# alshai/pfbwt-f

Hardware: AMD Instinct MI355X
Metric: Gbases/s end-to-end BWT+SA build; bit-exact .bwt/.sa vs reference (higher is better)
Workload: dtype u8 text / u32 indices / u64 hash; 1 GPU; S-32G; L=32000000, H=1000, seed=1000, w=10, p=100, flags=-r, uint_t=64, n=32000010000, r=83625322, input=text resident in HBM, outputs (.bwt, .ssa, .esa) left in HBM, per_rank=single GPU

## Files before the change

### include/pfbwt_hip_dev.h

```cpp
#ifndef PFBWT_HIP_DEV_H
#define PFBWT_HIP_DEV_H
#include "pfbwt_hip.h"

#ifdef __cplusplus
extern "C" {
#endif

int pfp_profile_enable(pfp_ctx *ctx, int on);
int pfp_profile_select(pfp_ctx *ctx, const char *kernel_name);
int pfp_profile_reset(pfp_ctx *ctx);
int pfp_profile_get(pfp_ctx *ctx, int idx, const char **name, uint64_t *launches, double *ms, double *bytes);
int pfp_stage_ms(pfp_ctx *ctx, double out[3]);
int pfp_debug_set(pfp_ctx *ctx, const char *key, long long value);
int pfp_debug_sort(pfp_ctx *ctx, uint64_t n, int bits, int reps, double *ms_out, uint32_t *unsorted_pairs, uint32_t *wrong_values);

int pfp_debug_prims_geometry(uint32_t out[4]);
int pfp_debug_sort_pairs(pfp_ctx *ctx, const void *keys, int key_bytes, const uint32_t *vals, uint64_t n, const int *ranges, int nranges,
                         void *keys_out, uint32_t *vals_out, uint32_t *guards_changed);
int pfp_debug_scan(pfp_ctx *ctx, const void *in, int elem_bytes, int op, int mode, uint64_t n, void *out, void *total, uint32_t *guards_changed);
int pfp_debug_compact(pfp_ctx *ctx, const uint32_t *in, const uint32_t *flag, uint64_t n, uint32_t *out, uint32_t *count, uint32_t *guards_changed);
int pfp_debug_checksum(pfp_ctx *ctx, const void *d_buf, uint64_t bytes, uint64_t global_offset, uint64_t out[2]);

int pfp_debug_check_sample_order(pfp_ctx *ctx, uint64_t out[5]);
int pfp_debug_check_sa(pfp_ctx *ctx, uint64_t out[5]);
int pfp_debug_check_samples(pfp_ctx *ctx, uint64_t out[3]);
int pfp_debug_rows_windowed(pfp_ctx *ctx, uint64_t window_rows, void *host_sa, void *host_lcp);
int pfp_debug_wordsum(pfp_ctx *ctx, const void *d_buf, uint64_t bytes, uint64_t out[2]);

#ifdef __cplusplus
}
#endif
#endif
```

### pfbwt-f_amd/csrc/common.h

```cpp
#pragma once
#include <hip/hip_runtime.h>
#include <cstdint>
#include <cstdio>
#include <cstdlib>
#include <cstring>
#include <chrono>
#include <string>
#include <vector>
#include "../../include/pfbwt_hip.h"
#include "devmem.h"
#include "../../include/pfbwt_hip_dev.h"

namespace pfp {

typedef uint32_t idx_t;

constexpr int BLOCK = 256;
constexpr int WAVE = 64;

constexpr uint8_t Dollar = 2, EndOfWord = 1, EndOfDict = 0;

enum KernelId {
    K_TRIGGER_SCAN, K_PHRASE_ENDS, K_PHRASE_HASH, K_PHRASE_HASH_LONG, K_DEDUP_HEADS, K_DEDUP_LONG,
    K_DICT_BUILD, K_RADIX_HIST, K_RADIX_SCATTER, K_SCAN_REDUCE, K_SCAN_SPINE, K_SCAN_APPLY,
// ... 157 lines not shown
    pfp::ResultSlot ms; uint64_t ms_patterns = 0, ms_bases = 0;
    std::vector<uint64_t> ms_off;
    pfp::ResultSlot rii; pfp::RiIndex rix;
    pfp::ResultSlot ri; uint64_t ri_patterns = 0, ri_reported = 0; int ri_route = 0;
    std::vector<uint64_t> ri_off;
    pfp::ResultSlot mem; uint64_t mem_patterns = 0, mem_count = 0;
    pfp::ResultSlot meml; uint64_t mem_reported = 0;
    std::vector<uint64_t> mem_off, mem_poff;
    size_t lo_after_parse = 0, lo_after_pbwt = 0, emit_scratch_mark = 0;
    bool prof_on = false; uint64_t prof_mask = ~0ULL;
    pfp::ProfRec prof[pfp::K_COUNT_];
    struct PendingEv { hipEvent_t a, b; int id; double bytes; };
    std::vector<PendingEv> pending;
    std::vector<hipEvent_t> ev_pool;
    double stage_ms[3] = {0, 0, 0};
    int hip_err = 0;
    uint8_t *hstage[2] = {nullptr, nullptr}; hipEvent_t hstage_ev[2] = {nullptr, nullptr}; bool hstage_used[2] = {false, false};
    pfp::Tunables tun;
    struct FastaIngest {
        uint8_t *raw[2] = {nullptr, nullptr}; size_t rawcap = 0; bool used[2] = {false, false};
        hipStream_t copy = nullptr; bool copy_ready = false; hipEvent_t ev_copied[2] = {nullptr, nullptr}, ev_free[2] = {nullptr, nullptr};
        uint8_t *tiles = nullptr; size_t tiles_cap = 0;
        unsigned long long *d_tot = nullptr, *h_tot = nullptr;
        uint32_t state = 2; bool started = false; uint64_t records = 0;
        std::vector<uint64_t> rec_raw, rec_pos;
    } fa;
    uint8_t *h_bwt = nullptr; void *h_sa = nullptr;
    uint8_t *ing_buf[16] = {};
    uint64_t ing_next_off = 0;
    std::vector<std::string> doc_names; std::vector<uint64_t> doc_starts;
    uint64_t hash_seed = 0x9E3779B97F4A7C15ULL;
    int num_cus = 0;
    uint32_t *d_trigtab = nullptr;
};

namespace pfp {

inline hipEvent_t ev_get(pfp_ctx *c)
{
    if (!c->ev_pool.empty()) { hipEvent_t e = c->ev_pool.back(); c->ev_pool.pop_back(); return e; }
    hipEvent_t e; (void)hipEventCreate(&e); return e;
}
inline void prof_collect(pfp_ctx *c)
{
    if (c->pending.empty()) return;
    (void)hipStreamSynchronize(c->stream);
    for (auto &pe : c->pending) {
        float ms = 0; (void)hipEventElapsedTime(&ms, pe.a, pe.b);
        c->prof[pe.id].launches++; c->prof[pe.id].ms += ms; c->prof[pe.id].bytes += pe.bytes;
        c->ev_pool.push_back(pe.a); c->ev_pool.push_back(pe.b);
    }
    c->pending.clear();
}
struct ProfScope {
    pfp_ctx *c; int id; double bytes; hipEvent_t a = nullptr; bool on = false;
    ProfScope(pfp_ctx *c_, int id_, double bytes_) : c(c_), id(id_), bytes(bytes_)
    {
        on = c->prof_on && ((c->prof_mask >> id) & 1ULL);
        if (on) { a = ev_get(c); (void)hipEventRecord(a, c->stream); }
    }
    ~ProfScope()
    {
        if (on) {
            hipEvent_t b = ev_get(c); (void)hipEventRecord(b, c->stream);
            c->pending.push_back({a, b, id, bytes});
            if (c->pending.size() > 4096) prof_collect(c);
// ... 68 lines not shown
```

### pfbwt-f_amd/csrc/emit.h

```cpp
#pragma once
#include "prims.h"
#include "parse.h"

namespace pfp {

__global__ __launch_bounds__(BLOCK) void k_pbwt_pack(const uint32_t *P, const uint8_t *last, const tpos_t *sai, uint64_t m, uint4 *rec)
{
    const uint64_t j = (uint64_t)blockIdx.x * BLOCK + threadIdx.x;
    if (j >= m) return;
    const uint64_t v = sai ? (uint64_t)sai[j] : 0ULL;
    rec[j] = make_uint4((uint32_t)v, (uint32_t)(v >> 32), P[j], (uint32_t)last[j ? j - 1 : m - 1]);
}
constexpr int BWL_SHIFT = 29;
__device__ __forceinline__ uint32_t bwl_code(uint32_t c) { return c == 0 ? 0u : c == Dollar ? 1u : c == '-' ? 2u : c == 'A' ? 3u : c == 'C' ? 4u : c == 'G' ? 5u : c == 'N' ? 6u : c == 'T' ? 7u : 8u; }
__device__ __forceinline__ uint8_t bwl_byte(uint32_t code) { return code == 0 ? (uint8_t)0 : code == 1 ? Dollar : code == 2 ? (uint8_t)'-' : code == 3 ? (uint8_t)'A' : code == 4 ? (uint8_t)'C' : code == 5 ? (uint8_t)'G' : code == 6 ? (uint8_t)'N' : (uint8_t)'T'; }
__global__ __launch_bounds__(BLOCK) void k_pbwt_rows(const uint32_t *SAP, const uint4 *rec, uint64_t m, uint8_t *bwlast, tpos_t *bwsai, uint32_t *W, uint32_t *rowid, int pack, uint32_t *bad)
{
    const uint64_t i = (uint64_t)blockIdx.x * BLOCK + threadIdx.x;
    if (i > m) return;
    const uint32_t s = SAP[i];
    if (s == 0) { bwlast[i] = 0; if (bwsai) bwsai[i] = 0; W[i] = 0; rowid[i] = (uint32_t)i; return; }
    const uint4 R = rec[s - 1];
    bwlast[i] = (uint8_t)R.w;
    if (bwsai) bwsai[i] = (tpos_t)(((uint64_t)R.y << 32) | R.x);
// ... 103 lines not shown
    const uint32_t *srank = nullptr;
    const tpos_t *bwsai = nullptr;
    const uint2 *posinfo = nullptr;
    const uint4 *prec = nullptr;
    const uint32_t *wordid = nullptr;
    int use_prec = 0;
    int use_e0 = 0;
    const uint4 *winfo = nullptr;
    const uint8_t *bwlast = nullptr;
    const uint8_t *bwl_il = nullptr;
    const tpos_t *bwsai_il = nullptr;
    const void *EB = nullptr;
    const uint32_t *s_sl = nullptr;
    const uint32_t *s_fb = nullptr;
    const uint8_t *s_fl = nullptr;
    const uint8_t *s_pc = nullptr;
    const uint32_t *s_g0 = nullptr;
    const uint32_t *gk = nullptr;
    const void *cnt = nullptr;
    const uint4 *sinfo = nullptr;
    const uint32_t *tile_slot = nullptr;
    uint64_t *big_keys = nullptr; uint32_t *big_vals = nullptr; unsigned long long *big_count = nullptr;
    uint64_t big_cap = 0, big_total = 0;
    uint64_t nout = 0, n = 0;
    uint64_t e0 = 0, e1 = 0;
    uint64_t w0 = 0, w1 = 0;
    const void *ENB = nullptr; const uint32_t *etile_slot = nullptr, *elist = nullptr, *cpos = nullptr; uint32_t ecount = 0; int special = 0; uint64_t q0 = 0;
    const uint32_t *qspec = nullptr;
    const uint32_t *gqf = nullptr, *gql = nullptr;
    uint8_t *gleft = nullptr, *tile_left = nullptr; uint32_t group_rows_cap = 0; uint32_t rank_members_max = 0;
    const uint4 *cinfo = nullptr;
    const unsigned long long *cgb = nullptr;
    const uint32_t *town = nullptr;
    uint32_t *lglist = nullptr; unsigned long long *lgcount = nullptr; uint64_t lgcap = 0; int qpasses = 0 ;
    unsigned long long *gstat = nullptr;
};
constexpr uint8_t SF_MULTI = 1, SF_FULL = 2, SF_BIG = 4, SF_GFULL = 8, SF_NONUNI = 16, SF_E0 = 32;
__device__ __forceinline__ bool slot_is_special(uint32_t fl) { return (fl & (SF_FULL | SF_GFULL | SF_NONUNI)) != 0; }
constexpr int EG_SLOTS = 2 * BLOCK;
constexpr uint32_t BIG_GROUP_MEMBERS = 64;
constexpr uint32_t WID_MASK = 0x0FFFFFFFu;
__device__ __forceinline__ uint32_t dict_code4(uint32_t c) { return c <= 2 ? c : (c == '-') ? 3u : (c == 'A') ? 4u : (c == 'C') ? 5u : (c == 'G') ? 6u : (c == 'N') ? 7u : 8u; }
__device__ __forceinline__ uint8_t dict_byte4(uint32_t code) { return code <= 2 ? (uint8_t)code : code == 3 ? (uint8_t)'-' : code == 4 ? (uint8_t)'A' : code == 5 ? (uint8_t)'C' : code == 6 ? (uint8_t)'G' : code == 7 ? (uint8_t)'N' : (uint8_t)'T'; }
__global__ __launch_bounds__(BLOCK) void k_pack_winfo(const uint32_t *ws, const uint32_t *wrank , const uint32_t *occ, const uint32_t *F, uint64_t dwords, uint4 *winfo)
{
    const uint64_t id = (uint64_t)blockIdx.x * BLOCK + threadIdx.x;
    if (id >= dwords) return;
    const uint32_t rk = wrank ? wrank[id] : (uint32_t)id;
    winfo[id] = make_uint4(ws[id], ws[id + 1] - 1u, F[rk], occ[rk]);
}
__global__ __launch_bounds__(BLOCK) void k_pack_posinfo(const uint8_t *D, const uint32_t *wordid, uint64_t dsize, uint2 *posinfo)
{
    const uint64_t x = (uint64_t)blockIdx.x * BLOCK + threadIdx.x;
    if (x >= dsize) return;
    posinfo[x] = make_uint2(wordid[x] | (dict_code4(x ? D[x - 1] : 0u) << 28), 0u);
}

constexpr uint32_t PREC_SL_BITS = 26, PREC_FULL = 1u << 30, PREC_VALID = 1u << 31;
__global__ __launch_bounds__(BLOCK) void k_pack_prec(const uint8_t *D, const uint32_t *wordid, const uint4 *winfo, uint64_t dsize, uint32_t dwords, uint4 *prec, const tpos_t *bwsai_il )
{
    const uint64_t x = (uint64_t)blockIdx.x * BLOCK + threadIdx.x;
    if (x >= dsize) return;
    const uint32_t id = wordid[x];
    uint4 R = make_uint4(0u, 0u, 0u, 0u);
    if (id < dwords) {
        const uint4 W = winfo[id];
        uint32_t code = 0, full = 0;
// ... 619 lines not shown
            }
        }
#pragma unroll
        for (int it = 0; it < EG_PER_THREAD; ++it) {
            const uint32_t r = threadIdx.x + (uint32_t)it * BLOCK;
            if (r < nrows) { LQ[r] = qv[it]; const uint32_t fl = s_kf[sv[it]] >> 24; if (fl & SF_MULTI) cv[it] = s_pc[sv[it]]; else if (!a.bwl_il) cv[it] = a.bwlast[qv[it]]; }
        }
        __syncthreads();
#pragma unroll
        for (int it = 0; it < EG_PER_THREAD; ++it) {
            const uint32_t r = threadIdx.x + (uint32_t)it * BLOCK;
            if (r < nrows) {
                const uint32_t s = sv[it], kf = s_kf[s];
                uint32_t pos = r;
                if ((kf >> 24) & SF_MULTI) {
                    const uint32_t sh = s - s_dl[s], k = kf & 0xFFFFFFu, q = qv[it];
                    uint32_t before = 0;
                    for (uint32_t mm = 0; mm < k; ++mm) {
                        const uint32_t sm = sh + mm;
                        if (sm != s) before += lower_bound_u32(LQ + s_eb[sm], s_eb[sm + 1] - s_eb[sm], q);
                    }
                    pos = s_eb[sh] + before + (r - s_eb[s]);
                }
                if (qrow) qrow[B0 - a.q0 + pos] = qv[it];
                const uint64_t o = s_ob[s] + pos;
                if (o >= a.w0 && o < a.w1) bwt[o - a.w0] = cv[it];
            }
        }
        __syncthreads();
        j += cut;
    }
}

template <int ITEMS> __device__ __forceinline__ void lds_sort_pairs_u32(uint32_t *keys, uint16_t *vals, uint32_t n, int npass, uint32_t (*wh)[RS_RADIX], uint32_t *red)
{
    const int lane = threadIdx.x & 63, wave = threadIdx.x >> 6;
    const uint32_t nit = (n + BLOCK - 1) / BLOCK;
    for (uint32_t j = n + threadIdx.x; j < nit * BLOCK; j += BLOCK) { keys[j] = 0xFFFFFFFFu; vals[j] = 0; }
    const uint32_t base = (uint32_t)wave * (nit * WAVE) + lane;
    for (int p = 0; p < npass; ++p) {
        const int sh = 8 * p;
        uint32_t k[ITEMS], dg[ITEMS]; uint16_t v[ITEMS];
#pragma unroll
        for (int w = 0; w < BLOCK / WAVE; ++w) wh[w][threadIdx.x] = 0;
        __syncthreads();
#pragma unroll
        for (int it = 0; it < ITEMS; ++it) {
            if ((uint32_t)it < nit) {
                const uint32_t i = base + (uint32_t)it * WAVE;
                k[it] = keys[i]; v[it] = vals[i];
                const uint32_t d = (k[it] >> sh) & 255u;
                uint32_t plo = 0xFFFFFFFFu, phi = 0xFFFFFFFFu;
                same_digit_lanes(d, plo, phi);
                const int leader = plo ? __builtin_ctz(plo) : 32 + __builtin_ctz(phi);
                uint32_t old = 0;
                if (lane == leader) { old = wh[wave][d]; wh[wave][d] = old + (uint32_t)__builtin_popcount(plo) + (uint32_t)__builtin_popcount(phi); }
                old = __shfl(old, leader);
                dg[it] = d | ((old + __builtin_amdgcn_mbcnt_hi(phi, __builtin_amdgcn_mbcnt_lo(plo, 0u))) << 8);
            }
        }
        __syncthreads();
        {
            const unsigned d = threadIdx.x;
            uint32_t cw[BLOCK / WAVE]; uint32_t total = 0;
#pragma unroll
            for (int w = 0; w < BLOCK / WAVE; ++w) { cw[w] = wh[w][d]; total += cw[w]; }
            uint32_t tt;
            uint32_t run = block_excl_sum(total, red, &tt);
#pragma unroll
            for (int w = 0; w < BLOCK / WAVE; ++w) { wh[w][d] = run; run += cw[w]; }
        }
        __syncthreads();
#pragma unroll
        for (int it = 0; it < ITEMS; ++it) {
            if ((uint32_t)it < nit) { const uint32_t li = wh[wave][dg[it] & 255u] + (dg[it] >> 8); keys[li] = k[it]; vals[li] = v[it]; }
        }
        __syncthreads();
    }
}
template <typename EBT, int BUF> __global__ __launch_bounds__(BLOCK) void k_emit_groups_large(EmitArgs a, uint8_t *bwt, uint32_t *qrow)
{
    __shared__ uint32_t LQ[BUF];
    __shared__ uint16_t LS[BUF];
    __shared__ uint32_t wh[BLOCK / WAVE][RS_RADIX];
    __shared__ uint32_t s_eb[EG_SLOTS + 1], s_fb[EG_SLOTS];
    __shared__ uint8_t s_pc[EG_SLOTS];
    __shared__ uint32_t red[4];
    const EBT *ENB = reinterpret_cast<const EBT *>(a.ENB);
    constexpr int WHICH = BUF > EG1_BUF ? 1 : 0;
    const unsigned long long have = a.lgcount[WHICH];
    const uint64_t cnt = have < a.lgcap ? have : a.lgcap;
    for (uint64_t g = blockIdx.x; g < cnt; g += gridDim.x) {
        const uint64_t j = a.lglist[(uint64_t)WHICH * a.lgcap + g];
        const uint32_t k = a.cinfo[j].y;
        const uint64_t B0 = (uint64_t)ENB[j], outbase = (uint64_t)a.cgb[j];
        for (uint32_t s = threadIdx.x; s < k; s += BLOCK) {
            const uint4 ci = a.cinfo[j + s];
            s_eb[s] = (uint32_t)((uint64_t)ENB[j + s] - B0); s_fb[s] = ci.x; s_pc[s] = (uint8_t)ci.w;
            if (s + 1 == k) s_eb[k] = (uint32_t)((uint64_t)ENB[j + k] - B0);
        }
        __syncthreads();
        const uint32_t nrows = s_eb[k];
        for (uint32_t r = threadIdx.x; r < nrows; r += BLOCK) { const uint32_t s = upper_bound_t<uint32_t>(s_eb, k, r) - 1u; LQ[r] = a.ilist[s_fb[s] + (r - s_eb[s])]; LS[r] = (uint16_t)s; }
        __syncthreads();
        lds_sort_pairs_u32<BUF / BLOCK>(LQ, LS, nrows, a.qpasses, wh, red);
        for (uint32_t r = threadIdx.x; r < nrows; r += BLOCK) {
            if (qrow) qrow[B0 - a.q0 + r] = LQ[r];
            const uint64_t o = outbase + r;
            if (o >= a.w0 && o < a.w1) bwt[o - a.w0] = s_pc[LS[r]];
        }
        __syncthreads();
    }
}

template <typename EBT> __global__ __launch_bounds__(BLOCK) void k_slice_bounds(EmitArgs a, uint64_t lo, uint64_t hi, unsigned long long *out)
{
    if (blockIdx.x != 0 || threadIdx.x != 0) return;
    const EBT *EB = reinterpret_cast<const EBT *>(a.EB);
    const EBT *ENB = reinterpret_cast<const EBT *>(a.ENB);
    const uint32_t il = slot_of_row<EBT>(a, lo);
    const uint32_t gh = (a.s_fl[il] & SF_MULTI) ? a.s_g0[il] : il;
    out[0] = EB[gh];
    out[2] = a.special ? (unsigned long long)ENB[a.cpos[gh]] : 0ULL;
    out[4] = a.special ? (unsigned long long)a.cpos[gh] : 0ULL;
    if (hi >= a.nout) { out[1] = a.nout; out[3] = a.special ? (unsigned long long)ENB[a.ecount] : 0ULL; out[5] = a.special ? (unsigned long long)a.ecount : 0ULL; return; }
    uint32_t s = slot_of_row<EBT>(a, hi - 1);
    if (a.s_fl[s] & SF_MULTI) { const uint32_t g = a.s_g0[s]; while (s < a.dsize && (a.s_fl[s] & SF_MULTI) && a.s_g0[s] == g) ++s; }
    else ++s;
    {
        uint64_t lo_ = s, hi_ = a.dsize;
        while (lo_ < hi_) { const uint64_t mid = lo_ + ((hi_ - lo_) >> 1); if ((uint64_t)EB[mid] < hi) lo_ = mid + 1; else hi_ = mid; }
        s = (uint32_t)lo_;
    }
    out[1] = s < a.dsize ? (uint64_t)EB[s] : a.nout;
    const uint32_t js = a.special ? (s < a.dsize ? a.cpos[s] : a.ecount) : 0u;
    out[3] = a.special ? (unsigned long long)ENB[js] : 0ULL; out[5] = js;
}

#ifndef PFP_FILL_NT
// ... 288 lines not shown
```

### pfbwt-f_amd/csrc/emit_host.h

```cpp
#pragma once

__global__ __launch_bounds__(BLOCK) void k_flag_special(const uint8_t *s_fl, uint64_t dsize, uint32_t *flag)
{
    const uint64_t i = (uint64_t)blockIdx.x * BLOCK + threadIdx.x;
    if (i < dsize) flag[i] = slot_is_special(s_fl[i]) ? 1u : 0u;
}
template <typename EBT> __global__ __launch_bounds__(BLOCK) void k_gather_counts(const EBT *cnt, const uint32_t *list, uint64_t n, EBT *out)
{
    const uint64_t j = (uint64_t)blockIdx.x * BLOCK + threadIdx.x;
    if (j < n) out[j] = cnt[list[j]];
}

struct EmitVisit { uint64_t window_rows; std::function<int(uint64_t first_row, uint64_t rows, const void *d_sa_window)> fn; };
struct EmitWin { uint64_t cs, ce, cl, e0, e1, q0, q1, j0, j1; };
static uint64_t slice_first_row(uint64_t total, int slice, int nslices)
{
    const uint64_t k = (uint64_t)nslices, s = (uint64_t)slice;
    return total / k * s + (total % k) * s / k;
}
static void print_left_rows(const unsigned long long *d_gstat)
{
    unsigned long long h[12];
    if (hipMemcpy(h, d_gstat, 96, hipMemcpyDeviceToHost) != hipSuccess) return;
    fprintf(stderr, "[pfbwt_hip] special rows left to the row-wise kernel (counted once per window that enumerates them): whole-word member %llu, sort route %llu, too many rows %llu, too many slots %llu; by group rows (<1K <4K <16K <64K <256K <1M <4M more):",
// ... 59 lines not shown
        }
        if (windowed) {
            unsigned long long *d_bounds; PFP_ALLOC_HI(c, d_bounds, unsigned long long, 6 * nchunks);
            for (uint64_t ch = 0; ch < nchunks; ++ch)
                PFP_LAUNCH(c, K_MISC, 64, (k_slice_bounds<EBT>), 1, ea, wins[(size_t)ch].cs - wins[(size_t)ch].cl, wins[(size_t)ch].ce, d_bounds + 6 * ch);
            std::vector<unsigned long long> hb(6 * (size_t)nchunks);
            PFP_HIP(c, hipMemcpyAsync(hb.data(), d_bounds, hb.size() * 8, hipMemcpyDeviceToHost, c->stream));
            PFP_HIP(c, hipStreamSynchronize(c->stream));
            for (uint64_t ch = 0; ch < nchunks; ++ch) { EmitWin &wn = wins[(size_t)ch]; const unsigned long long *b = &hb[6 * (size_t)ch]; wn.e0 = b[0]; wn.e1 = b[1]; wn.q0 = b[2]; wn.q1 = b[3]; wn.j0 = b[4]; wn.j1 = b[5]; }
        }
        for (const EmitWin &wn : wins) { if (wn.q1 - wn.q0 > maxq) maxq = wn.q1 - wn.q0; if (wn.ce - wn.cs > maxrows) maxrows = wn.ce - wn.cs; }
        return PFP_OK;
    }

    int alloc_routes()
    {
        if (ea.big_total) {
            if (ea.big_total >= 0xFFFFFFF0ULL) return PFP_E_TOO_LARGE;
            PFP_ALLOC_HI(c, bk0, uint64_t, ea.big_total); PFP_ALLOC_HI(c, bk1, uint64_t, ea.big_total);
            PFP_ALLOC_HI(c, bv0, uint32_t, ea.big_total); PFP_ALLOC_HI(c, bv1, uint32_t, ea.big_total); PFP_ALLOC_HI(c, btg, uint32_t, ea.big_total);
        }
        ea.big_keys = bk0; ea.big_vals = bv0; ea.big_count = d_b + 4; ea.big_cap = ea.big_total;
        ea.group_rows_cap = c->tun.emit_group_rows; ea.rank_members_max = c->tun.big_group_members != -2 ? 0xFFFFFFFFu : c->tun.emit_group_rows >= (uint32_t)EG_BUF ? BIG_GROUP_MEMBERS : 3u;
        const uint64_t max_etiles = maxq / EMIT_TILE + 3;
        if (runaware && ea.group_rows_cap && tot2 && ea.cinfo) {
            PFP_ALLOC_HI(c, ea.gleft, uint8_t, (size_t)ea.ecount + 1); PFP_ALLOC_HI(c, ea.tile_left, uint8_t, max_etiles);
            PFP_HIP(c, hipMemsetAsync(ea.gleft, 0, (size_t)ea.ecount + 1, c->stream));
        }
        ea.qpasses = (bits_for(c->nrows ? c->nrows : 0xFFFFFFFFULL) + 7) / 8;
        if (ea.gleft) {
            const uint32_t cap = ea.group_rows_cap < (uint32_t)EG_BUF ? ea.group_rows_cap : (uint32_t)EG_BUF;
            ea.lgcap = maxq / cap + 2;
            PFP_ALLOC_HI(c, ea.lglist, uint32_t, 2 * ea.lgcap); PFP_ALLOC_HI(c, ea.lgcount, unsigned long long, 2);
        }
        if (ea.gleft && c->tun.verbose) { PFP_ALLOC_HI(c, ea.gstat, unsigned long long, 12); PFP_HIP(c, hipMemsetAsync(ea.gstat, 0, 96, c->stream)); }
        return PFP_OK;
    }

    int emit_window(const EmitWin &wn, uint8_t *bwt_at, SAT *sa_at, uint32_t *q_at, bool fill)
    {
        ea.w0 = wn.cs - wn.cl; ea.w1 = wn.ce;
        if (ea.big_total) PFP_HIP(c, hipMemsetAsync(ea.big_count, 0, 16, c->stream));
        if (runaware) PFP_TRY(emit_runaware(wn, bwt_at, q_at, fill));
        else PFP_TRY(emit_all_rows(wn, bwt_at, sa_at, q_at));
        return ea.big_total ? place_big_groups(bwt_at, sa_at, q_at) : PFP_OK;
    }
    int emit_runaware(const EmitWin &wn, uint8_t *bwt_at, uint32_t *q_at, bool fill)
    {
        ea.e0 = wn.q0; ea.e1 = wn.q1; ea.q0 = wn.q0;
        if (fill) {
            const uint32_t fill_subs = c->tun.fill_subs < 1u ? 1u : c->tun.fill_subs > FILL_MAX_SUBS ? FILL_MAX_SUBS : c->tun.fill_subs;
            const uint64_t super = (uint64_t)FILL_GROUPS * FILL_SUB;
            const uint64_t nsub = (ea.w1 - 1) / super - ea.w0 / super + 1;
            const int skip = c->tun.fill_skip ? 1 : 0;
            if (fill_masks) PFP_LAUNCH(c, K_FILL, (ea.w1 - ea.w0) * 9 / 8, (k_fill<EBT, true>), nblocks(nsub, fill_subs), ea, bwt_at, fill_subs, skip, rmask, wn.cs);
            else PFP_LAUNCH(c, K_FILL, ea.w1 - ea.w0, (k_fill<EBT, false>), nblocks(nsub, fill_subs), ea, bwt_at, fill_subs, skip, (uint16_t *)nullptr, (uint64_t)0);
        }
        if (ea.e1 <= ea.e0) return PFP_OK;
        const unsigned ge = (unsigned)((ea.e1 - 1) / EMIT_TILE - ea.e0 / EMIT_TILE + 1);
        if (ea.gleft) {
            PFP_HIP(c, hipMemsetAsync(ea.tile_left, 0, (size_t)ge, c->stream));
            PFP_HIP(c, hipMemsetAsync(ea.lgcount, 0, 16, c->stream));
            PFP_LAUNCH(c, K_EMIT, (ea.e1 - ea.e0) * (1 + 4 + (q_at ? 4 : 0)), (k_emit_groups<EBT>), ge, ea, bwt_at, q_at);
            PFP_LAUNCH(c, K_EMIT_LARGE, 0, (k_emit_groups_large<EBT, EG1_BUF>), ge < 1024u ? ge : 1024u, ea, bwt_at, q_at);
            PFP_LAUNCH(c, K_EMIT_LARGE, 0, (k_emit_groups_large<EBT, EG2_BUF>), ge < 512u ? ge : 512u, ea, bwt_at, q_at);
            PFP_LAUNCH(c, K_EMIT_BIG, 0, (k_emit<SAT, EBT>), ge, ea, bwt_at, (SAT *)nullptr, q_at);
        } else
            PFP_LAUNCH(c, K_EMIT, (ea.e1 - ea.e0) * (1 + 4 + (q_at ? 4 : 0)), (k_emit<SAT, EBT>), ge, ea, bwt_at, (SAT *)nullptr, q_at);
        return PFP_OK;
    }
    int emit_all_rows(const EmitWin &wn, uint8_t *bwt_at, SAT *sa_at, uint32_t *q_at)
    {
        ea.e0 = wn.e0; ea.e1 = wn.e1; ea.q0 = 0;
        PFP_LAUNCH(c, K_EMIT, (ea.w1 - ea.w0) * (1 + 4 + (sa_at ? 8 + sizeof(SAT) : 0) + (q_at ? 4 : 0)),
                   (k_emit<SAT, EBT>), (unsigned)((ea.e1 - 1) / EMIT_TILE - ea.e0 / EMIT_TILE + 1), ea, bwt_at, sa_at, q_at);
        return PFP_OK;
    }
    int place_big_groups(uint8_t *bwt_at, SAT *sa_at, uint32_t *q_at)
    {
        unsigned long long hb[2];
        PFP_HIP(c, hipMemcpyAsync(hb, ea.big_count, 16, hipMemcpyDeviceToHost, c->stream));
        PFP_HIP(c, hipStreamSynchronize(c->stream));
        if (hb[1] || hb[0] > ea.big_total) return PFP_E_CORRUPT;
        const uint64_t nb = hb[0];
        if (!nb) return PFP_OK;
        const BitRange big_ranges[2] = {{0, bits_for(c->nrows)}, {32, 32 + bits_for(ea.dsize)}};
        uint64_t *sk; uint32_t *sv;
        PFP_TRY(radix_sort_pairs<uint64_t>(c, bk0, bv0, bk1, bv1, nb, big_ranges, 2, &sk, &sv));
        PFP_LAUNCH(c, K_EMIT_BIG, nb * 12, k_big_heads, nblocks(nb, BLOCK), (const uint64_t *)sk, nb, btg);
        PFP_TRY((device_scan<uint32_t, 1>(c, btg, btg, nb, nullptr)));
        PFP_LAUNCH(c, K_EMIT_BIG, nb * (30 + sizeof(SAT)), (k_big_place<SAT, EBT>), nblocks(nb, BLOCK), ea, (const uint64_t *)sk, (const uint32_t *)sv, (const uint32_t *)btg, nb, bwt_at, sa_at, q_at);
        return PFP_OK;
    }

    int stream_out(const EmitWin &wn)
    {
        if (!c->h_bwt && !c->h_sa) return PFP_OK;
        const uint64_t r0 = wn.cs - wn.cl < s0 ? s0 : wn.cs - wn.cl, r1 = wn.ce == s1 ? wn.ce : wn.ce - 1;
// ... 409 lines not shown
```

### pfbwt-f_amd/csrc/pfbwt_hip.hip

```cpp
#include "common.h"
#include "prims.h"
#include "parse.h"
#include "fasta.h"
#include "sufsort.h"
#include "recsort.h"
#include "dictrec.h"
#include "emit.h"
#include "markers.h"
#include "docarray.h"
#include "lcparray.h"
#include "thresholds.h"
#include "matchstats.h"
#include "runindex.h"
#include "mems.h"
#include <algorithm>
#include <functional>
#include <map>
#include <sched.h>
#include <thread>
#if defined(__SSE2__)
#include <emmintrin.h>
#endif

using namespace pfp;
// ... 165 lines not shown
    pfp_ctx *c = nullptr;
    if (w < 1 || w > 32 || p == 0) st = PFP_E_ARG;
    else {
        int ndev = 0;
        if (hipGetDeviceCount(&ndev) != hipSuccess || ndev <= 0 || device < 0 || device >= ndev) st = PFP_E_HIP;
        else if (hipSetDevice(device) != hipSuccess) st = PFP_E_HIP;
        else {
            c = new pfp_ctx();
            c->w = w; c->p = p; c->flags = flags; c->device = device; c->arena_request = (size_t)workspace_bytes;
            load_tunables_from_env(c);
            if (hipStreamCreateWithFlags(&c->stream, hipStreamNonBlocking) != hipSuccess) { delete c; c = nullptr; st = PFP_E_HIP; }
        }
    }
    if (status) *status = st;
    return c;
}

void pfp_destroy(pfp_ctx *c)
{
    if (!c) return;
    (void)hipSetDevice(c->device);
    if (c->stream) (void)hipStreamSynchronize(c->stream);
    (void)hipDeviceSynchronize();
    prof_collect(c);
    for (auto e : c->ev_pool) (void)hipEventDestroy(e);
    c->text.destroy();
    for (int k = 0; k < 2; ++k) { if (c->fa.raw[k]) (void)hipFree(c->fa.raw[k]); if (c->fa.ev_copied[k]) (void)hipEventDestroy(c->fa.ev_copied[k]); if (c->fa.ev_free[k]) (void)hipEventDestroy(c->fa.ev_free[k]); }
    if (c->fa.tiles) (void)hipFree(c->fa.tiles);
    if (c->fa.d_tot) (void)hipFree(c->fa.d_tot);
    if (c->fa.h_tot) (void)hipHostFree(c->fa.h_tot);
    if (c->fa.copy_ready) (void)hipStreamDestroy(c->fa.copy);
    for (auto &q : c->ing_buf) if (q) (void)hipHostFree(q);
    if (c->d_trigtab) (void)hipFree(c->d_trigtab);
    for (int k = 0; k < 2; ++k) { if (c->hstage[k]) (void)hipHostFree(c->hstage[k]); if (c->hstage_ev[k]) (void)hipEventDestroy(c->hstage_ev[k]); }
    c->arena.vm.destroy();
    if (c->stream) (void)hipStreamDestroy(c->stream);
    delete c;
}

int pfp_error_detail(pfp_ctx *c, uint64_t *pos, int *ch)
{
    if (!c) return PFP_E_ARG;
    if (pos) *pos = c->err_pos;
    if (ch) *ch = c->err_ch;
    return PFP_OK;
}
uint64_t pfp_workspace_needed(pfp_ctx *c) { return c ? (uint64_t)(c->arena.cap + c->arena.want) : 0; }
int pfp_reset(pfp_ctx *c)
{
    if (!c) return PFP_E_ARG;
    PFP_HIP(c, hipSetDevice(c->device));
    PFP_HIP(c, hipStreamSynchronize(c->stream));
    reset_results(c);
    return PFP_OK;
}

int pfp_profile_enable(pfp_ctx *c, int on) { if (!c) return PFP_E_ARG; prof_collect(c); c->prof_on = on != 0; c->prof_mask = ~0ULL; return PFP_OK; }
int pfp_profile_select(pfp_ctx *c, const char *kernel)
{
    if (!c || !kernel) return PFP_E_ARG;
    prof_collect(c);
    for (int i = 0; i < K_COUNT_; ++i) if (!strcmp(kernel, kernel_names[i])) { c->prof_on = true; c->prof_mask = 1ULL << i; return PFP_OK; }
    return PFP_E_ARG;
}
int pfp_profile_reset(pfp_ctx *c) { if (!c) return PFP_E_ARG; prof_collect(c); for (auto &r : c->prof) r = ProfRec(); return PFP_OK; }
int pfp_profile_get(pfp_ctx *c, int idx, const char **name, uint64_t *launches, double *ms, double *bytes)
// ... 1461 lines not shown
    uint64_t *k0, *k1; uint32_t *v0, *v1, *d_bad;
    PFP_ALLOC_HI(c, k0, uint64_t, n); PFP_ALLOC_HI(c, k1, uint64_t, n); PFP_ALLOC_HI(c, v0, uint32_t, n); PFP_ALLOC_HI(c, v1, uint32_t, n); PFP_ALLOC_HI(c, d_bad, uint32_t, 2);
    BitRange br = {0, bits};
    double best = 1e30;
    uint64_t *sk = k0; uint32_t *sv = v0;
    for (int r = 0; r < reps; ++r) {
        PFP_LAUNCH(c, K_MISC, n * 12, k_debug_fill, nblocks(n, BLOCK), k0, v0, n, bits, (uint64_t)r * 7919);
        PFP_HIP(c, hipStreamSynchronize(c->stream));
        HostTimer t;
        int rc = radix_sort_pairs<uint64_t>(c, k0, v0, k1, v1, n, &br, 1, &sk, &sv);
        if (rc != PFP_OK) return rc;
        PFP_HIP(c, hipStreamSynchronize(c->stream));
        const double ms = t.ms();
        if (ms < best) best = ms;
    }
    PFP_HIP(c, hipMemsetAsync(d_bad, 0, 8, c->stream));
    PFP_LAUNCH(c, K_MISC, n * 12, k_debug_check_sorted, nblocks(n, BLOCK), (const uint64_t *)sk, (const uint32_t *)sv, n, bits, (uint64_t)(reps - 1) * 7919, d_bad);
    uint32_t bad[2] = {0, 0};
    PFP_HIP(c, hipMemcpyAsync(bad, d_bad, 8, hipMemcpyDeviceToHost, c->stream));
    PFP_HIP(c, hipStreamSynchronize(c->stream));
    if (ms_out) *ms_out = best;
    if (unsorted_pairs) *unsorted_pairs = bad[0];
    if (wrong_values) *wrong_values = bad[1];
    c->arena.reset();
    return PFP_OK;
}

int pfp_debug_prims_geometry(uint32_t out[4])
{
    if (!out) return PFP_E_ARG;
    out[0] = (uint32_t)RS_TILE; out[1] = (uint32_t)SCAN_TILE; out[2] = SEG_SMALL_MAX; out[3] = (uint32_t)Tunables().seg_grid;
    return PFP_OK;
}
namespace pfp {
extern "C++" {
constexpr size_t DEBUG_GUARD = 256;
constexpr uint8_t DEBUG_GUARD_BYTE = 0xA5;
struct GuardedBuf { char *raw = nullptr; size_t bytes = 0; template <typename T> T *data() const { return (T *)(raw + DEBUG_GUARD); } };
static int guarded_alloc(pfp_ctx *c, size_t bytes, uint8_t fill, GuardedBuf *g)
{
    g->raw = (char *)c->arena.alloc_hi(bytes + 2 * DEBUG_GUARD); g->bytes = bytes;
    if (!g->raw) return PFP_E_NOMEM;
    PFP_HIP(c, hipMemsetAsync(g->raw, DEBUG_GUARD_BYTE, DEBUG_GUARD, c->stream));
    if (bytes) PFP_HIP(c, hipMemsetAsync(g->raw + DEBUG_GUARD, fill, bytes, c->stream));
    PFP_HIP(c, hipMemsetAsync(g->raw + DEBUG_GUARD + bytes, DEBUG_GUARD_BYTE, DEBUG_GUARD, c->stream));
    return PFP_OK;
}
static int guards_check(pfp_ctx *c, const GuardedBuf &g, uint32_t *changed)
{
    uint8_t h[2 * DEBUG_GUARD];
    PFP_HIP(c, hipMemcpyAsync(h, g.raw, DEBUG_GUARD, hipMemcpyDeviceToHost, c->stream));
    PFP_HIP(c, hipMemcpyAsync(h + DEBUG_GUARD, g.raw + DEBUG_GUARD + g.bytes, DEBUG_GUARD, hipMemcpyDeviceToHost, c->stream));
    PFP_HIP(c, hipStreamSynchronize(c->stream));
    uint32_t bad = 0; size_t first = 0;
    for (size_t i = 0; i < 2 * DEBUG_GUARD; ++i) if (h[i] != DEBUG_GUARD_BYTE && !bad++) first = i;
    if (bad && c->tun.verbose) fprintf(stderr, "[pfbwt_hip] guard of the %zu-byte buffer at arena offset %zu (arena %p + %zu): %u bytes changed, the first %s the data at guard byte %zu: %02x\n", g.bytes,
                                       c->arena.offset_of(g.raw), (void *)c->arena.base, c->arena.cap, bad, first < DEBUG_GUARD ? "in front of" : "behind", first % DEBUG_GUARD, h[first]);
    *changed += bad;
    return PFP_OK;
}
template <typename K> static int debug_sort_pairs(pfp_ctx *c, const K *keys, const uint32_t *vals, uint64_t n, const BitRange *ranges, int nranges, K *keys_out, uint32_t *vals_out, uint32_t *changed)
{
    GuardedBuf k[2], v[2];
    for (int i = 0; i < 2; ++i) { PFP_TRY(guarded_alloc(c, n * sizeof(K), 0xEE, &k[i])); PFP_TRY(guarded_alloc(c, n * 4, 0xEE, &v[i])); }
    if (n) {
        PFP_HIP(c, hipMemcpyAsync(k[0].data<K>(), keys, n * sizeof(K), hipMemcpyHostToDevice, c->stream));
// ... 234 lines not shown
```

### pfbwt-f_amd/python/pfbwt_hip.py

```python
import ctypes as C
import os
import numpy as np

_HERE = os.path.dirname(os.path.abspath(__file__))
DEFAULT_LIB = os.path.join(os.path.dirname(_HERE), "lib", "libpfbwt_hip.so")

PFP_OK = 0
FLAG_U64, FLAG_NON_ACGT_TO_A, FLAG_SAI = 1, 2, 4
DA_ROWS, DA_RUNS = 1, 2
LCP_ROWS, LCP_RUNS = 1, 2
E_ARG = -1
E_INVALID_CHAR, E_TOO_LARGE, E_NOMEM, E_HIP, E_ONE_WORD, E_STATE, E_CORRUPT = -2, -3, -4, -5, -6, -7, -8


class PfpError(RuntimeError):
    def __init__(self, status, msg, pos=None, ch=None):
        super().__init__("pfbwt_hip: %s (status %d)" % (msg, status))
        self.status, self.pos, self.ch = status, pos, ch


class ParseSizes(C.Structure):
    _fields_ = [("n", C.c_uint64), ("m", C.c_uint64), ("dwords", C.c_uint64), ("dsize", C.c_uint64)]


# ... 72 lines not shown
    L.pfp_bwt_device_ptrs.argtypes = [vp, C.POINTER(vp), C.POINTER(vp), C.POINTER(vp), C.POINTER(vp)]
    L.pfp_shard_view_get.argtypes = [vp, C.POINTER(ShardView)]
    L.pfp_parse_feed_left_context.argtypes = [vp]
    L.pfp_shard_load.argtypes = [vp, vp, u64, vp, u64]
    L.pfp_device_copy.argtypes = [vp, vp, vp, u64]
    L.pfp_merge_shards.argtypes = [vp, i32, C.POINTER(ShardView), C.POINTER(ParseSizes)]
    L.pfp_sacak_int_u32.argtypes = [vp, vp, C.c_uint32, C.c_uint32]
    L.pfp_sacak_int_u64.argtypes = [vp, vp, u64, u64]
    L.pfp_marker_array.argtypes = [vp, vp, u64, vp, u64, C.POINTER(u64)]
    L.pfp_marker_array_get.argtypes = [vp, vp]
    L.pfp_gsacak_u32.argtypes = [vp, vp, vp, vp, C.c_uint32]
    L.pfp_gsacak_u64.argtypes = [vp, vp, vp, vp, u64]
    L.pfp_profile_enable.argtypes = [vp, i32]
    L.pfp_profile_reset.argtypes = [vp]
    L.pfp_profile_select.argtypes = [vp, C.c_char_p]
    L.pfp_profile_get.argtypes = [vp, i32, C.POINTER(C.c_char_p), C.POINTER(u64), C.POINTER(C.c_double), C.POINTER(C.c_double)]
    L.pfp_stage_ms.argtypes = [vp, C.POINTER(C.c_double)]
    L.pfp_debug_set.argtypes = [vp, C.c_char_p, C.c_longlong]
    L.pfp_parse_feed_fasta.argtypes = [vp, vp, u64, C.c_uint, C.POINTER(u64)]
    L.pfp_parse_fasta_records.argtypes = [vp, vp, vp]
    L.pfp_parse_reserve.argtypes = [vp, u64]
    L.pfp_parse_feed_fasta_file.argtypes = [vp, C.c_char_p, C.c_uint, C.POINTER(IngestInfo)]
    L.pfp_bwt_build_stream.argtypes = [vp, i32, i32, vp, vp, C.POINTER(BwtSizes)]
    L.pfp_text_length.argtypes = [vp, C.POINTER(u64)]
    L.pfp_bwt_get_expanded.argtypes = [vp, vp, vp, i32]
    L.pfp_text_view.argtypes = [vp, C.POINTER(vp), C.POINTER(u64)]
    L.pfp_host_register.argtypes = [vp, u64]
    L.pfp_host_unregister.argtypes = [vp]
    L.pfp_debug_wordsum.argtypes = [vp, vp, u64, C.POINTER(u64)]
    L.pfp_debug_check_sample_order.argtypes = [vp, C.POINTER(u64)]
    L.pfp_debug_check_sa.argtypes = [vp, C.POINTER(u64)]
    L.pfp_parse_feed_device_view.argtypes = [vp, vp, u64, u64, u64]
    L.pfp_debug_check_samples.argtypes = [vp, C.POINTER(u64)]
    L.pfp_sharded_create.restype = vp
    L.pfp_sharded_create.argtypes = [i32, u64, C.c_uint, i32, C.POINTER(i32), u64, C.POINTER(i32)]
    L.pfp_sharded_destroy.argtypes = [vp]; L.pfp_sharded_destroy.restype = None
    L.pfp_sharded_ctx.restype = vp; L.pfp_sharded_ctx.argtypes = [vp, i32]
    L.pfp_sharded_ranks.argtypes = [vp]
    L.pfp_sharded_build.argtypes = [vp, i32, i32, vp, vp, C.POINTER(u64), C.POINTER(u64), C.POINTER(u64)]
    L.pfp_sharded_reset.argtypes = [vp]
    L.pfp_sharded_error.restype = C.c_char_p; L.pfp_sharded_error.argtypes = [vp]
    L.pfp_parse_docs.argtypes = [vp, C.POINTER(u64)]
    L.pfp_parse_doc_get.argtypes = [vp, u64, C.POINTER(C.c_char_p), C.POINTER(u64)]
    L.pfp_doc_array.argtypes = [vp, vp, u64, C.c_uint]
    L.pfp_doc_array_get.argtypes = [vp, vp, vp, vp]
    L.pfp_doc_array_device_ptrs.argtypes = [vp, C.POINTER(vp), C.POINTER(vp), C.POINTER(vp)]
    L.pfp_doc_array_write.argtypes = [vp, i32, i32, i32]
    L.pfp_lcp_array.argtypes = [vp, C.c_uint, C.POINTER(LcpInfo)]
    L.pfp_lcp_array_get.argtypes = [vp, vp, vp]
    L.pfp_lcp_array_device_ptrs.argtypes = [vp, C.POINTER(vp), C.POINTER(vp)]
    L.pfp_lcp_array_write.argtypes = [vp, i32, i32]
    L.pfp_thresholds.argtypes = [vp, C.POINTER(ThrInfo)]
    L.pfp_thresholds_get.argtypes = [vp, vp, vp]
    L.pfp_thresholds_device_ptrs.argtypes = [vp, C.POINTER(vp), C.POINTER(vp)]
    L.pfp_thresholds_write.argtypes = [vp, i32, i32]
    L.pfp_thresholds_windowed.argtypes = [vp, u64, C.POINTER(ThrInfo), C.POINTER(u64)]
    L.pfp_debug_rows_windowed.argtypes = [vp, u64, vp, vp]
    L.pfp_ms_index.argtypes = [vp]
    L.pfp_ms_query.argtypes = [vp, vp, vp, u64, C.POINTER(MsInfo)]
    L.pfp_ms_query_file.argtypes = [vp, C.c_char_p, C.POINTER(MsInfo)]
    L.pfp_ms_offsets_get.argtypes = [vp, vp, C.POINTER(u64)]
    L.pfp_ms_get.argtypes = [vp, vp, vp]
    L.pfp_ms_device_ptrs.argtypes = [vp, C.POINTER(vp), C.POINTER(vp)]
    L.pfp_ms_write.argtypes = [vp, i32, i32]
    L.pfp_ri_index.argtypes = [vp]
    L.pfp_ri_count.argtypes = [vp, vp, vp, u64, C.POINTER(RiInfo)]
# ... 74 lines not shown
        ro = np.empty(nrec.value, np.uint64); tp = np.empty(nrec.value, np.uint64)
        self._check(self.L.pfp_parse_fasta_records(self.h, _ptr(ro), _ptr(tp)))
        return ro, tp

    def feed_fasta_file(self, path, records=False):
        info = IngestInfo()
        self._check(self.L.pfp_parse_feed_fasta_file(self.h, os.fsencode(path), 2 if records else 0, C.byref(info)))
        return info

    def text_length(self):
        n = C.c_uint64(0); self._check(self.L.pfp_text_length(self.h, C.byref(n))); return n.value

    def bwt_build_stream(self, host_bwt_ptr, host_sa_ptr=None, rssa=False):
        b = BwtSizes()
        self._check(self.L.pfp_bwt_build_stream(self.h, 1 if host_sa_ptr else 0, 1 if rssa else 0, C.c_void_p(host_bwt_ptr), C.c_void_p(host_sa_ptr) if host_sa_ptr else None, C.byref(b)))
        self.bsizes, self._want, self._rows, self.esa_pairs = b, (bool(host_sa_ptr), bool(rssa)), b.nout, b.r
        return b

    def check_sample_order(self):
        o = (C.c_uint64 * 5)()
        self._check(self.L.pfp_debug_check_sample_order(self.h, o))
        return {"pairs": int(o[0]), "order_violations": int(o[1]), "rows_not_adjacent": int(o[2]), "max_lcp": int(o[3]), "mean_lcp": (int(o[4]) / int(o[0])) if o[0] else 0.0}

    def check_sa(self):
        o = (C.c_uint64 * 5)()
        self._check(self.L.pfp_debug_check_sa(self.h, o))
        return {"rows": int(o[0]), "out_of_range": int(o[1]), "duplicates": int(o[2]), "bwt_mismatches": int(o[3]), "eos_bytes": int(o[4])}

    def check_samples(self):
        o = (C.c_uint64 * 3)()
        self._check(self.L.pfp_debug_check_samples(self.h, o))
        return {"runs": int(o[0]), "row_errors": int(o[1]), "value_errors": int(o[2])}

    def bwt_get_expanded(self, host_bwt_ptr, ssa=None, threads=16):
        self._check(self.L.pfp_bwt_get_expanded(self.h, C.c_void_p(host_bwt_ptr), _ptr(ssa), int(threads)))

    def samples_get(self, out=None):
        b = self.bsizes
        ssa = out["ssa"] if out else np.empty(2 * b.r, self.udt); esa = out["esa"] if out else np.empty(2 * b.r, self.udt)
        self._check(self.L.pfp_bwt_get(self.h, None, None, _ptr(ssa), _ptr(esa)))
        return ssa, esa

    def feed_host_batch(self, host_ptr, count, length, stride):
        self._check(self.L.pfp_parse_feed_batch(self.h, C.c_void_p(int(host_ptr)), int(count), int(length), int(stride)))

    def feed_device_view(self, dptr, count, length, stride):
        self._check(self.L.pfp_parse_feed_device_view(self.h, C.c_void_p(int(dptr)), int(count), int(length), int(stride)))

    def feed_device(self, dptr, nbytes, end_of_seq=True):
        self._check(self.L.pfp_parse_feed_device(self.h, C.c_void_p(int(dptr)), int(nbytes), 1 if end_of_seq else 0))

    def finalize(self, shard=False):
        s = ParseSizes()
        self._check((self.L.pfp_parse_finalize_shard if shard else self.L.pfp_parse_finalize)(self.h, C.byref(s)))
        self.sizes = s
        return s

    def parse_get(self):
        s = self.sizes
        out = {"dict": np.empty(s.dsize, np.uint8), "occ": np.empty(s.dwords, self.udt), "parse": np.empty(s.m, np.uint32),
               "last": np.empty(s.m, np.uint8), "sai": np.empty(s.m, self.udt) if self.sai else None}
        self._check(self.L.pfp_parse_get(self.h, _ptr(out["dict"]), _ptr(out["occ"]), _ptr(out["parse"]), _ptr(out["last"]), _ptr(out["sai"])))
        return out

    def parse_bwt(self):
        self._check(self.L.pfp_parse_bwt(self.h))
# ... 359 lines not shown
```

Before: 140.1 Gbases/s.

## Widen large-group emit kernels to 512/1024 threads and pack sort payload

The large-group emit kernels now run with 512 and 1024 threads per workgroup instead of 256, and their grid caps are derived from the CU count instead of being fixed. The LDS radix sort is made generic over thread count and packs the member index into the digit/rank register, saving a per-item register array. A debug counter of large groups taken is added, which costs one atomic per launch. The aim is more parallelism per large group's LDS sort, at the risk of lower occupancy and heavier barriers.

```diff
diff --git a/include/pfbwt_hip_dev.h b/include/pfbwt_hip_dev.h
--- a/include/pfbwt_hip_dev.h
+++ b/include/pfbwt_hip_dev.h
@@ -15,6 +15,7 @@
 int pfp_debug_sort(pfp_ctx *ctx, uint64_t n, int bits, int reps, double *ms_out, uint32_t *unsorted_pairs, uint32_t *wrong_values);
 
 int pfp_debug_prims_geometry(uint32_t out[4]);
+int pfp_debug_emit_large_groups(pfp_ctx *ctx, uint64_t out[4]);
 int pfp_debug_sort_pairs(pfp_ctx *ctx, const void *keys, int key_bytes, const uint32_t *vals, uint64_t n, const int *ranges, int nranges,
                          void *keys_out, uint32_t *vals_out, uint32_t *guards_changed);
 int pfp_debug_scan(pfp_ctx *ctx, const void *in, int elem_bytes, int op, int mode, uint64_t n, void *out, void *total, uint32_t *guards_changed);
diff --git a/pfbwt-f_amd/csrc/common.h b/pfbwt-f_amd/csrc/common.h
--- a/pfbwt-f_amd/csrc/common.h
+++ b/pfbwt-f_amd/csrc/common.h
@@ -213,6 +213,7 @@
     uint64_t hash_seed = 0x9E3779B97F4A7C15ULL;
     int num_cus = 0;
     uint32_t *d_trigtab = nullptr;
+    unsigned long long *d_lgtaken = nullptr;
 };
 
 namespace pfp {
diff --git a/pfbwt-f_amd/csrc/emit.h b/pfbwt-f_amd/csrc/emit.h
--- a/pfbwt-f_amd/csrc/emit.h
+++ b/pfbwt-f_amd/csrc/emit.h
@@ -159,7 +159,7 @@
     const uint4 *cinfo = nullptr;
     const unsigned long long *cgb = nullptr;
     const uint32_t *town = nullptr;
-    uint32_t *lglist = nullptr; unsigned long long *lgcount = nullptr; uint64_t lgcap = 0; int qpasses = 0 ;
+    uint32_t *lglist = nullptr; unsigned long long *lgcount = nullptr, *lgtaken = nullptr ; uint64_t lgcap = 0; int qpasses = 0 ;
     unsigned long long *gstat = nullptr;
 };
 constexpr uint8_t SF_MULTI = 1, SF_FULL = 2, SF_BIG = 4, SF_GFULL = 8, SF_NONUNI = 16, SF_E0 = 32;
@@ -845,23 +845,46 @@
     }
 }
 
-template <int ITEMS> __device__ __forceinline__ void lds_sort_pairs_u32(uint32_t *keys, uint16_t *vals, uint32_t n, int npass, uint32_t (*wh)[RS_RADIX], uint32_t *red)
+#ifndef PFP_EGL1_THREADS
+#define PFP_EGL1_THREADS 512
+#endif
+#ifndef PFP_EGL2_THREADS
+#define PFP_EGL2_THREADS 1024
+#endif
+constexpr int EGL1_THREADS = PFP_EGL1_THREADS, EGL2_THREADS = PFP_EGL2_THREADS;
+constexpr int EGL1_WG_PER_CU = 2, EGL2_WG_PER_CU = 1;
+__device__ __forceinline__ uint32_t digits_excl_sum(uint32_t v, uint32_t *red)
 {
     const int lane = threadIdx.x & 63, wave = threadIdx.x >> 6;
-    const uint32_t nit = (n + BLOCK - 1) / BLOCK;
-    for (uint32_t j = n + threadIdx.x; j < nit * BLOCK; j += BLOCK) { keys[j] = 0xFFFFFFFFu; vals[j] = 0; }
+    uint32_t inc = 0;
+    if (wave < RS_RADIX / WAVE) { inc = wave_incl_sum(v); if (lane == 63) red[wave] = inc; }
+    __syncthreads();
+    uint32_t base = 0;
+#pragma unroll
+    for (int i = 0; i < RS_RADIX / WAVE; ++i) if (i < wave) base += red[i];
+    return base + inc - v;
+}
+template <int ITEMS, int THREADS> __device__ __forceinline__ void lds_sort_pairs_u32(uint32_t *keys, uint16_t *vals, uint32_t n, int npass, uint32_t (*wh)[RS_RADIX], uint32_t *red)
+{
+    constexpr int NW = THREADS / WAVE;
+    static_assert(THREADS % WAVE == 0 && THREADS >= RS_RADIX, "threads 0 .. 255 own a digit each");
+    static_assert(ITEMS * WAVE <= (1 << 14) && EG_SLOTS <= (1 << 9), "digit, rank and member share a word");
+    const int lane = threadIdx.x & 63, wave = threadIdx.x >> 6;
+    const uint32_t nit = (n + THREADS - 1) / THREADS;
+    for (uint32_t j = n + threadIdx.x; j < nit * THREADS; j += THREADS) { keys[j] = 0xFFFFFFFFu; vals[j] = 0; }
     const uint32_t base = (uint32_t)wave * (nit * WAVE) + lane;
     for (int p = 0; p < npass; ++p) {
         const int sh = 8 * p;
-        uint32_t k[ITEMS], dg[ITEMS]; uint16_t v[ITEMS];
-#pragma unroll
-        for (int w = 0; w < BLOCK / WAVE; ++w) wh[w][threadIdx.x] = 0;
+        uint32_t k[ITEMS], pk[ITEMS];
+#pragma unroll
+        for (int w = 0; w < NW * RS_RADIX / THREADS; ++w) (&wh[0][0])[threadIdx.x + w * THREADS] = 0;
         __syncthreads();
 #pragma unroll
         for (int it = 0; it < ITEMS; ++it) {
             if ((uint32_t)it < nit) {
                 const uint32_t i = base + (uint32_t)it * WAVE;
-                k[it] = keys[i]; v[it] = vals[i];
+                k[it] = keys[i];
+                const uint32_t mem = vals[i];
                 const uint32_t d = (k[it] >> sh) & 255u;
                 uint32_t plo = 0xFFFFFFFFu, phi = 0xFFFFFFFFu;
                 same_digit_lanes(d, plo, phi);
@@ -869,55 +892,61 @@
                 uint32_t old = 0;
                 if (lane == leader) { old = wh[wave][d]; wh[wave][d] = old + (uint32_t)__builtin_popcount(plo) + (uint32_t)__builtin_popcount(phi); }
                 old = __shfl(old, leader);
-                dg[it] = d | ((old + __builtin_amdgcn_mbcnt_hi(phi, __builtin_amdgcn_mbcnt_lo(plo, 0u))) << 8);
+                pk[it] = d | ((old + __builtin_amdgcn_mbcnt_hi(phi, __builtin_amdgcn_mbcnt_lo(plo, 0u))) << 8) | (mem << 22);
             }
         }
         __syncthreads();
         {
-            const unsigned d = threadIdx.x;
-            uint32_t cw[BLOCK / WAVE]; uint32_t total = 0;
-#pragma unroll
-            for (int w = 0; w < BLOCK / WAVE; ++w) { cw[w] = wh[w][d]; total += cw[w]; }
-            uint32_t tt;
-            uint32_t run = block_excl_sum(total, red, &tt);
-#pragma unroll
-            for (int w = 0; w < BLOCK / WAVE; ++w) { wh[w][d] = run; run += cw[w]; }
+            const unsigned d = threadIdx.x & (RS_RADIX - 1);
+            const bool own = threadIdx.x < (unsigned)RS_RADIX;
+            uint32_t cw[NW]; uint32_t total = 0;
+            if (own) {
+#pragma unroll
+                for (int w = 0; w < NW; ++w) { cw[w] = wh[w][d]; total += cw[w]; }
+            }
+            uint32_t run = digits_excl_sum(total, red);
+            if (own) {
+#pragma unroll
+                for (int w = 0; w < NW; ++w) { wh[w][d] = run; run += cw[w]; }
+            }
         }
         __syncthreads();
 #pragma unroll
         for (int it = 0; it < ITEMS; ++it) {
-            if ((uint32_t)it < nit) { const uint32_t li = wh[wave][dg[it] & 255u] + (dg[it] >> 8); keys[li] = k[it]; vals[li] = v[it]; }
-        }
-        __syncthreads();
-    }
-}
-template <typename EBT, int BUF> __global__ __launch_bounds__(BLOCK) void k_emit_groups_large(EmitArgs a, uint8_t *bwt, uint32_t *qrow)
-{
+            if ((uint32_t)it < nit) { const uint32_t li = wh[wave][pk[it] & 255u] + ((pk[it] >> 8) & 0x3FFFu); keys[li] = k[it]; vals[li] = (uint16_t)(pk[it] >> 22); }
+        }
+        __syncthreads();
+    }
+}
+template <typename EBT, int BUF, int THREADS> __global__ __launch_bounds__(THREADS) void k_emit_groups_large(EmitArgs a, uint8_t *bwt, uint32_t *qrow)
+{
+    static_assert(BUF % THREADS == 0 && (THREADS / WAVE * RS_RADIX) % THREADS == 0, "whole items per thread, whole counters per thread");
     __shared__ uint32_t LQ[BUF];
     __shared__ uint16_t LS[BUF];
-    __shared__ uint32_t wh[BLOCK / WAVE][RS_RADIX];
+    __shared__ uint32_t wh[THREADS / WAVE][RS_RADIX];
     __shared__ uint32_t s_eb[EG_SLOTS + 1], s_fb[EG_SLOTS];
     __shared__ uint8_t s_pc[EG_SLOTS];
-    __shared__ uint32_t red[4];
+    __shared__ uint32_t red[RS_RADIX / WAVE];
     const EBT *ENB = reinterpret_cast<const EBT *>(a.ENB);
     constexpr int WHICH = BUF > EG1_BUF ? 1 : 0;
     const unsigned long long have = a.lgcount[WHICH];
     const uint64_t cnt = have < a.lgcap ? have : a.lgcap;
+    if (a.lgtaken && blockIdx.x == 0 && threadIdx.x == 0) atomicAdd(a.lgtaken + WHICH, (unsigned long long)cnt);
     for (uint64_t g = blockIdx.x; g < cnt; g += gridDim.x) {
         const uint64_t j = a.lglist[(uint64_t)WHICH * a.lgcap + g];
         const uint32_t k = a.cinfo[j].y;
         const uint64_t B0 = (uint64_t)ENB[j], outbase = (uint64_t)a.cgb[j];
-        for (uint32_t s = threadIdx.x; s < k; s += BLOCK) {
+        for (uint32_t s = threadIdx.x; s < k; s += THREADS) {
             const uint4 ci = a.cinfo[j + s];
             s_eb[s] = (uint32_t)((uint64_t)ENB[j + s] - B0); s_fb[s] = ci.x; s_pc[s] = (uint8_t)ci.w;
             if (s + 1 == k) s_eb[k] = (uint32_t)((uint64_t)ENB[j + k] - B0);
         }
         __syncthreads();
         const uint32_t nrows = s_eb[k];
-        for (uint32_t r = threadIdx.x; r < nrows; r += BLOCK) { const uint32_t s = upper_bound_t<uint32_t>(s_eb, k, r) - 1u; LQ[r] = a.ilist[s_fb[s] + (r - s_eb[s])]; LS[r] = (uint16_t)s; }
-        __syncthreads();
-        lds_sort_pairs_u32<BUF / BLOCK>(LQ, LS, nrows, a.qpasses, wh, red);
-        for (uint32_t r = threadIdx.x; r < nrows; r += BLOCK) {
+        for (uint32_t r = threadIdx.x; r < nrows; r += THREADS) { const uint32_t s = upper_bound_t<uint32_t>(s_eb, k, r) - 1u; LQ[r] = a.ilist[s_fb[s] + (r - s_eb[s])]; LS[r] = (uint16_t)s; }
+        __syncthreads();
+        lds_sort_pairs_u32<BUF / THREADS, THREADS>(LQ, LS, nrows, a.qpasses, wh, red);
+        for (uint32_t r = threadIdx.x; r < nrows; r += THREADS) {
             if (qrow) qrow[B0 - a.q0 + r] = LQ[r];
             const uint64_t o = outbase + r;
             if (o >= a.w0 && o < a.w1) bwt[o - a.w0] = s_pc[LS[r]];
diff --git a/pfbwt-f_amd/csrc/emit_host.h b/pfbwt-f_amd/csrc/emit_host.h
--- a/pfbwt-f_amd/csrc/emit_host.h
+++ b/pfbwt-f_amd/csrc/emit_host.h
@@ -115,6 +115,9 @@
             const uint32_t cap = ea.group_rows_cap < (uint32_t)EG_BUF ? ea.group_rows_cap : (uint32_t)EG_BUF;
             ea.lgcap = maxq / cap + 2;
             PFP_ALLOC_HI(c, ea.lglist, uint32_t, 2 * ea.lgcap); PFP_ALLOC_HI(c, ea.lgcount, unsigned long long, 2);
+            if (!c->d_lgtaken) PFP_HIP(c, hipMalloc((void **)&c->d_lgtaken, 16));
+            PFP_HIP(c, hipMemsetAsync(c->d_lgtaken, 0, 16, c->stream));
+            ea.lgtaken = c->d_lgtaken;
         }
         if (ea.gleft && c->tun.verbose) { PFP_ALLOC_HI(c, ea.gstat, unsigned long long, 12); PFP_HIP(c, hipMemsetAsync(ea.gstat, 0, 96, c->stream)); }
         return PFP_OK;
@@ -145,8 +148,10 @@
             PFP_HIP(c, hipMemsetAsync(ea.tile_left, 0, (size_t)ge, c->stream));
             PFP_HIP(c, hipMemsetAsync(ea.lgcount, 0, 16, c->stream));
             PFP_LAUNCH(c, K_EMIT, (ea.e1 - ea.e0) * (1 + 4 + (q_at ? 4 : 0)), (k_emit_groups<EBT>), ge, ea, bwt_at, q_at);
-            PFP_LAUNCH(c, K_EMIT_LARGE, 0, (k_emit_groups_large<EBT, EG1_BUF>), ge < 1024u ? ge : 1024u, ea, bwt_at, q_at);
-            PFP_LAUNCH(c, K_EMIT_LARGE, 0, (k_emit_groups_large<EBT, EG2_BUF>), ge < 512u ? ge : 512u, ea, bwt_at, q_at);
+            const unsigned cus = c->num_cus > 0 ? (unsigned)c->num_cus : 256u;
+            const unsigned cap1 = 2u * EGL1_WG_PER_CU * cus, cap2 = 2u * EGL2_WG_PER_CU * cus;
+            PFP_LAUNCH_B(c, K_EMIT_LARGE, 0, (k_emit_groups_large<EBT, EG1_BUF, EGL1_THREADS>), ge < cap1 ? ge : cap1, EGL1_THREADS, ea, bwt_at, q_at);
+            PFP_LAUNCH_B(c, K_EMIT_LARGE, 0, (k_emit_groups_large<EBT, EG2_BUF, EGL2_THREADS>), ge < cap2 ? ge : cap2, EGL2_THREADS, ea, bwt_at, q_at);
             PFP_LAUNCH(c, K_EMIT_BIG, 0, (k_emit<SAT, EBT>), ge, ea, bwt_at, (SAT *)nullptr, q_at);
         } else
             PFP_LAUNCH(c, K_EMIT, (ea.e1 - ea.e0) * (1 + 4 + (q_at ? 4 : 0)), (k_emit<SAT, EBT>), ge, ea, bwt_at, (SAT *)nullptr, q_at);
diff --git a/pfbwt-f_amd/csrc/pfbwt_hip.hip b/pfbwt-f_amd/csrc/pfbwt_hip.hip
--- a/pfbwt-f_amd/csrc/pfbwt_hip.hip
+++ b/pfbwt-f_amd/csrc/pfbwt_hip.hip
@@ -221,6 +221,7 @@
     if (c->fa.copy_ready) (void)hipStreamDestroy(c->fa.copy);
     for (auto &q : c->ing_buf) if (q) (void)hipHostFree(q);
     if (c->d_trigtab) (void)hipFree(c->d_trigtab);
+    if (c->d_lgtaken) (void)hipFree(c->d_lgtaken);
     for (int k = 0; k < 2; ++k) { if (c->hstage[k]) (void)hipHostFree(c->hstage[k]); if (c->hstage_ev[k]) (void)hipEventDestroy(c->hstage_ev[k]); }
     c->arena.vm.destroy();
     if (c->stream) (void)hipStreamDestroy(c->stream);
@@ -1748,6 +1749,18 @@
     out[0] = (uint32_t)RS_TILE; out[1] = (uint32_t)SCAN_TILE; out[2] = SEG_SMALL_MAX; out[3] = (uint32_t)Tunables().seg_grid;
     return PFP_OK;
 }
+int pfp_debug_emit_large_groups(pfp_ctx *c, uint64_t out[4])
+{
+    if (!c || !out) return PFP_E_ARG;
+    out[0] = out[1] = 0; out[2] = (uint64_t)EG1_BUF; out[3] = (uint64_t)EG2_BUF;
+    if (!c->d_lgtaken) return PFP_OK;
+    PFP_HIP(c, hipSetDevice(c->device));
+    unsigned long long h[2];
+    PFP_HIP(c, hipMemcpyAsync(h, c->d_lgtaken, 16, hipMemcpyDeviceToHost, c->stream));
+    PFP_HIP(c, hipStreamSynchronize(c->stream));
+    out[0] = h[0]; out[1] = h[1];
+    return PFP_OK;
+}
 namespace pfp {
 extern "C++" {
 constexpr size_t DEBUG_GUARD = 256;
diff --git a/pfbwt-f_amd/python/pfbwt_hip.py b/pfbwt-f_amd/python/pfbwt_hip.py
--- a/pfbwt-f_amd/python/pfbwt_hip.py
+++ b/pfbwt-f_amd/python/pfbwt_hip.py
@@ -128,6 +128,8 @@
     L.pfp_debug_check_sa.argtypes = [vp, C.POINTER(u64)]
     L.pfp_parse_feed_device_view.argtypes = [vp, vp, u64, u64, u64]
     L.pfp_debug_check_samples.argtypes = [vp, C.POINTER(u64)]
+    if hasattr(L, "pfp_debug_emit_large_groups"):
+        L.pfp_debug_emit_large_groups.argtypes = [vp, C.POINTER(u64)]
     L.pfp_sharded_create.restype = vp
     L.pfp_sharded_create.argtypes = [i32, u64, C.c_uint, i32, C.POINTER(i32), u64, C.POINTER(i32)]
     L.pfp_sharded_destroy.argtypes = [vp]; L.pfp_sharded_destroy.restype = None
@@ -268,6 +270,11 @@
         self._check(self.L.pfp_debug_check_samples(self.h, o))
         return {"runs": int(o[0]), "row_errors": int(o[1]), "value_errors": int(o[2])}
 
+    def emit_large_groups(self):
+        o = (C.c_uint64 * 4)()
+        self._check(self.L.pfp_debug_emit_large_groups(self.h, o))
+        return {"groups_8k": int(o[0]), "groups_16k": int(o[1]), "rows_8k": int(o[2]), "rows_16k": int(o[3])}
+
     def bwt_get_expanded(self, host_bwt_ptr, ssa=None, threads=16):
         self._check(self.L.pfp_bwt_get_expanded(self.h, C.c_void_p(host_bwt_ptr), _ptr(ssa), int(threads)))
 
```

Result: faster. 144.0 Gbases/s, median of 6 (+2.8%).
